# superlinear-ai/raglite

Measured on AMD Instinct MI355X. Metric: queries/sec, MaxSim 32x1M d=1024 exact top-100, higher is better.
Workload: dtype f32 in / f32 scores: candidate chunks found with the fp16 hi halves of corpus and queries (1 x v_mfma_f32_16x16x32_f16 per multiply, f32 accumulate, rigorous error bound), their scores by v_mfma_f32_16x16x4_f32 (exact f32 products); full-precision fallback: 3 x v_mfma_f32_16x16x32_f16 on hi+lo pairs

## Files before the change

raglite_amd/csrc/maxsim_pp.hip:

```cpp
#include <cstdio>
#include <cstdlib>
#include <utility>

#include "common.h"
#include "pp_schedule.h"
#include "scratch_layout.h"

namespace rl {

typedef float f32x4 __attribute__((ext_vector_type(4)));
typedef _Float16 h16x8 __attribute__((ext_vector_type(8)));

namespace {
constexpr int PP_RT = 128;
constexpr int PP_NBLK = PP_RT / 16;
constexpr int PP_QPP = 16;
constexpr int PP_DC = 8;
constexpr int PP_LC = 6;
constexpr int PP_CSLOT = PP_NBLK * 1024;
constexpr int PP_STAGE = 1536;
constexpr int PP_LDS = PP_DC * PP_CSLOT + 16 * PP_STAGE * 4;

__device__ __forceinline__ int64_t pp_uniform_i64(int64_t v) {
    const uint32_t lo = __builtin_amdgcn_readfirstlane((uint32_t)(uint64_t)v);
    const uint32_t hi = __builtin_amdgcn_readfirstlane((uint32_t)((uint64_t)v >> 32));
    return (int64_t)(((uint64_t)hi << 32) | lo);
}

enum { PP_HINT_NONE = 0, PP_HINT_NT = 1, PP_HINT_SC1 = 2 };
template <bool NT>
__device__ __forceinline__ void pp_dma(uint32_t lds, const char* src, uint32_t lane16, int hint) {
    const uint32_t l = __builtin_amdgcn_readfirstlane(lds);
    const char* const p = reinterpret_cast<const char*>(pp_uniform_i64(reinterpret_cast<int64_t>(src)));
#ifdef RAGLITE_EXPERIMENTS
    if (!NT && hint == PP_HINT_SC1) {
        asm volatile("s_mov_b32 m0, %0\n\ts_nop 0\n\tglobal_load_lds_dwordx4 %1, %2 sc1" ::"s"(l), "v"(lane16), "s"(p) : "memory", "m0");
        return;
    }
    if (NT || hint == PP_HINT_NT)
#else
    if constexpr (NT)
#endif
        asm volatile("s_mov_b32 m0, %0\n\ts_nop 0\n\tglobal_load_lds_dwordx4 %1, %2 nt" ::"s"(l), "v"(lane16), "s"(p) : "memory", "m0");
    else
        asm volatile("s_mov_b32 m0, %0\n\ts_nop 0\n\tglobal_load_lds_dwordx4 %1, %2" ::"s"(l), "v"(lane16), "s"(p) : "memory", "m0");
}

template <int OFF>
__device__ __forceinline__ void pp_read(f32x4& dst, uint32_t addr) {
    asm volatile("ds_read_b128 %0, %1 offset:%2" : "=v"(dst) : "v"(addr), "n"(OFF) : "memory");
}
__device__ __forceinline__ void pp_pin(f32x4& a, f32x4& b, f32x4& c, f32x4& d) { asm volatile("" : "+v"(a), "+v"(b), "+v"(c), "+v"(d)); }
typedef float f32x16s __attribute__((ext_vector_type(16)));
__device__ __forceinline__ f32x16s pp_sload16(const float* p) {
    f32x16s v;
    const float* const u = reinterpret_cast<const float*>(pp_uniform_i64(reinterpret_cast<int64_t>(p)));
    asm volatile("s_load_dwordx16 %0, %1, 0x0\n\ts_waitcnt lgkmcnt(0)" : "=s"(v) : "s"(u) : "memory");
    return v;
}
__device__ __forceinline__ h16x8 pp_h(const f32x4& v) {
    h16x8 r;
    __builtin_memcpy(&r, &v, 16);
    return r;
}
}

struct PpRows {
    const float* tau;
    const float* q_unscale;
    const float* q_sumsq;
    const float* row_norm;
    const float* blk_minmax;
    int32_t B, QT, metric;
    float* cand_scores; int32_t* cand_ids; uint32_t* cand_cnt; uint32_t* overflow; int32_t cap;
    uint2* log; int32_t log_cap;
    int32_t tile_begin, tile_count;
    float* S; int64_t ld_s; int32_t stride;
    int32_t xcd_passes, dma_hint;
};

template <int DBG, int MODE, bool ROWNORM>
__global__ __launch_bounds__(512, 2) void maxsim_pp_kernel(const char* __restrict__ planes, int64_t n_rows, int32_t nslab,
                                                           const char* __restrict__ qfrag, const float* __restrict__ qmeta, int32_t n_q,
                                                           const int32_t* __restrict__ row_to_chunk, const int64_t* __restrict__ chunk_offsets,
                                                           const uint32_t* __restrict__ ends_bits, float* __restrict__ out, int64_t out_stride,
                                                           float inv_e_scale, const uint32_t* __restrict__ run_if, PpRows rs) {
    constexpr bool ROWS = MODE == 2, SCORES = MODE == 1, GROUPS = ROWS || SCORES;
    __shared__ __attribute__((aligned(16))) char smem[PP_LDS];
    if (run_if && __builtin_amdgcn_readfirstlane((int)*run_if) == 0) return;
    const int lane = threadIdx.x & 63;
    const int wv = wave_id();
    int64_t G = gridDim.x, b = blockIdx.x;
    int qt = (int)blockIdx.y;
    if constexpr (!GROUPS) {
        const int32_t passes = (n_q + PP_QPP - 1) / PP_QPP;
        const PpSlot m = gridDim.y > 1 ? pp_schedule((int32_t)blockIdx.x, (int32_t)blockIdx.y, (int32_t)gridDim.x, (int32_t)gridDim.y, passes)
                                       : pp_schedule_affine((int32_t)blockIdx.x, (int32_t)gridDim.x, passes, rs.xcd_passes);
        G = __builtin_amdgcn_readfirstlane(m.ranges);
        b = __builtin_amdgcn_readfirstlane(m.range);
        qt = __builtin_amdgcn_readfirstlane(m.pass);
    }
    auto boundary = [&](int64_t t) -> int64_t {
        if (t <= 0) return 0;
        if (t >= n_rows) return n_rows;
        const int32_t c = row_to_chunk[t];
        const int64_t c0 = chunk_offsets[c], c1 = chunk_offsets[c + 1];
        return c0 == t ? t : c1;
    };
    int32_t r_lo = 0, r_hi = 0, nt_rows = 0;
    if constexpr (!GROUPS) {
        r_lo = (int32_t)pp_uniform_i64(boundary((n_rows * b) / G));
        r_hi = (int32_t)pp_uniform_i64((b + 1 == G) ? n_rows : boundary((n_rows * (b + 1)) / G));
        if (r_hi <= r_lo) return;
    } else {
        const int64_t Tr = rs.tile_count;
        const int64_t t0 = (Tr * b) / G, t1 = (Tr * (b + 1)) / G;
        nt_rows = (int32_t)(t1 - t0);
        if (nt_rows <= 0) return;
        r_lo = (int32_t)((rs.tile_begin + t0) * PP_RT);
        r_hi = (int32_t)n_rows;
    }
    const int32_t org = r_lo & ~15;
    const int nt = GROUPS ? nt_rows : (r_hi - org + PP_RT - 1) / PP_RT;
    auto tile_blk = [&](int t) __attribute__((always_inline)) -> int32_t {
        if constexpr (SCORES) {
            const int32_t o = (org >> 7) + t;
            return ((o >> 1) * 2 * rs.stride + (o & 1)) * PP_NBLK;
        } else {
            return (org >> 4) + t * PP_NBLK;
        }
    };
    const int q_base = GROUPS ? 0 : PP_QPP * qt;
    const int total = nt * nslab;
    const int32_t last_blk = (int32_t)((n_rows + 15) >> 4) - 1;
    const uint32_t lds_base = (uint32_t)reinterpret_cast<uintptr_t>((__attribute__((address_space(3))) char*)smem);
    const uint32_t lane16 = 16u * lane;

    const bool has0 = q_base + 2 * wv < n_q, has1 = q_base + 2 * wv + 1 < n_q;
    int ql0 = PP_QPP * qt + 2 * wv, ql1 = PP_QPP * qt + 2 * wv + 1;
    ql0 = ql0 < n_q ? ql0 : n_q - 1;
    ql1 = ql1 < n_q ? ql1 : n_q - 1;
    const char* const qp0 = qfrag + pp_uniform_i64((int64_t)ql0 * nslab * 4096);
    const char* const qp1 = qfrag + pp_uniform_i64((int64_t)ql1 * nslab * 4096);
    int qr_s = 0;
    auto issue_qregs = [&](f32x4 (&qn)[4]) __attribute__((always_inline)) {
        if constexpr (!(DBG & 32)) {
            const char* const a0 = reinterpret_cast<const char*>(pp_uniform_i64(reinterpret_cast<int64_t>(qp0 + (int64_t)qr_s * 4096)));
            const char* const a1 = reinterpret_cast<const char*>(pp_uniform_i64(reinterpret_cast<int64_t>(qp1 + (int64_t)qr_s * 4096)));
            asm volatile("global_load_dwordx4 %0, %2, %3\n\tglobal_load_dwordx4 %1, %2, %3 offset:2048"
                         : "=&v"(qn[0]), "=&v"(qn[1]) : "v"(lane16), "s"(a0) : "memory");
            asm volatile("global_load_dwordx4 %0, %2, %3\n\tglobal_load_dwordx4 %1, %2, %3 offset:2048"
                         : "=&v"(qn[2]), "=&v"(qn[3]) : "v"(lane16), "s"(a1) : "memory");
            if (++qr_s == nslab) qr_s = 0;
        }
    };
    int fc_s = 0, fc_r = 0, fc_slot = 0;
    const int dma_hint = GROUPS ? 0 : rs.dma_hint;
    const int32_t blk_org = (org >> 4) + wv;
    const int64_t slab_bytes = (int64_t)nslab * 1024;
    auto issue_c = [&]() __attribute__((always_inline)) {
        if constexpr (!(DBG & 16)) {
            const int t = fc_r < nt ? fc_r : nt - 1;
            int32_t blk = SCORES ? tile_blk(t) + wv : blk_org + t * PP_NBLK;
            blk = blk < last_blk ? blk : last_blk;
            const char* src = planes + pp_uniform_i64((int64_t)blk * slab_bytes + (int64_t)fc_s * 1024);
            pp_dma<GROUPS>(lds_base + (uint32_t)(fc_slot * PP_CSLOT + wv * 1024), src, lane16, dma_hint);
        }
        if (++fc_s == nslab) { fc_s = 0; ++fc_r; }
        fc_slot = fc_slot + 1 == PP_DC ? 0 : fc_slot + 1;
    };

    f32x4 acc[2][2][PP_NBLK];
#pragma unroll
    for (int q = 0; q < 2; ++q)
#pragma unroll
        for (int qb = 0; qb < 2; ++qb)
#pragma unroll
            for (int a = 0; a < PP_NBLK; ++a) acc[q][qb][a] = (f32x4){0.f, 0.f, 0.f, 0.f};

    f32x4 ef[PP_NBLK];
    f32x4 qA[4], qB[4];
    int c_slot = 0;
    const uint32_t rd_c = lds_base + lane16;
    auto read_slab = [&](auto A_) __attribute__((always_inline)) {
        constexpr int a = decltype(A_)::value;
        if constexpr (!(DBG & 8)) pp_read<a * 1024>(ef[a], rd_c + (uint32_t)(c_slot * PP_CSLOT));
    };
    auto mfma_group = [&](f32x4 (&q)[4], auto A_) __attribute__((always_inline)) {
        constexpr int A = decltype(A_)::value;
        if constexpr (!(DBG & 2)) {
            acc[0][0][A] = __builtin_amdgcn_mfma_f32_16x16x32_f16(pp_h(ef[A]), pp_h(q[0]), acc[0][0][A], 0, 0, 0);
            acc[0][1][A] = __builtin_amdgcn_mfma_f32_16x16x32_f16(pp_h(ef[A]), pp_h(q[1]), acc[0][1][A], 0, 0, 0);
            acc[1][0][A] = __builtin_amdgcn_mfma_f32_16x16x32_f16(pp_h(ef[A]), pp_h(q[2]), acc[1][0][A], 0, 0, 0);
            acc[1][1][A] = __builtin_amdgcn_mfma_f32_16x16x32_f16(pp_h(ef[A]), pp_h(q[3]), acc[1][1][A], 0, 0, 0);
        }
    };

    const int fG = lane >> 4, fb = (lane >> 2) & 3, ft = lane & 3;
    const int my_row = (ft >> 1) + 2 * (fb & 1) + 4 * (fb >> 1) + 8 * (fG & 1);
    const uint32_t my_bit = 1u << my_row, my_below = my_bit - 1u;
    float run = -INFINITY;
    uint32_t prev_last_end = 1;
    int32_t ord_run = GROUPS ? 0 : __builtin_amdgcn_readfirstlane(row_to_chunk[org]);
    const int e_q = fG >> 1;
    const bool e_has = !GROUPS && (e_q == 0 ? has0 : has1) && (ft & 1) == 0;
    const float e_unscale = e_has ? qmeta[2 * (q_base + 2 * wv + e_q)] * inv_e_scale : 0.f;
    [[maybe_unused]] float* const o_buf = reinterpret_cast<float*>(smem + PP_DC * PP_CSLOT) + (2 * wv + e_q) * PP_STAGE;
    [[maybe_unused]] const int32_t ord_lo = !GROUPS ? __builtin_amdgcn_readfirstlane(row_to_chunk[r_lo]) : 0;
    [[maybe_unused]] int32_t own_cnt = 0, own_flushed = 0;
    [[maybe_unused]] auto flush_out = [&]() __attribute__((always_inline)) {
        if constexpr (!GROUPS) {
            const int n = own_cnt - own_flushed;
            asm volatile("s_waitcnt lgkmcnt(0)" ::: "memory");
            const float* const b0 = reinterpret_cast<const float*>(smem + PP_DC * PP_CSLOT) + (2 * wv) * PP_STAGE;
            float* const g0 = out + (int64_t)(q_base + 2 * wv) * out_stride + ord_lo + own_flushed;
            if (has0)
                for (int i = lane; i < n; i += 64) g0[i] = b0[i];
            if (has1)
                for (int i = lane; i < n; i += 64) g0[out_stride + i] = b0[PP_STAGE + i];
            own_flushed = own_cnt;
            asm volatile("s_waitcnt vmcnt(0)" ::: "memory");
        }
    };
    const uint64_t odd_pairs = 0xccccccccccccccccull;
    auto swap32 = [](float& x, float& y) __attribute__((always_inline)) {
        const auto r = __builtin_amdgcn_permlane32_swap(__float_as_uint(x), __float_as_uint(y), false, false);
        x = __uint_as_float(r[0]);
        y = __uint_as_float(r[1]);
    };
    auto swap16 = [](float& x, float& y) __attribute__((always_inline)) {
        const auto r = __builtin_amdgcn_permlane16_swap(__float_as_uint(x), __float_as_uint(y), false, false);
        x = __uint_as_float(r[0]);
        y = __uint_as_float(r[1]);
    };
    auto zero_block = [&](auto A_) __attribute__((always_inline)) {
        constexpr int a = decltype(A_)::value;
#pragma unroll
        for (int q = 0; q < 2; ++q)
#pragma unroll
            for (int qb = 0; qb < 2; ++qb) acc[q][qb][a] = (f32x4){0.f, 0.f, 0.f, 0.f};
    };
    [[maybe_unused]] auto block_epilogue_maxsim = [&](auto A_, int T) __attribute__((always_inline)) {
        constexpr int a = decltype(A_)::value;
        const int32_t base = org + T * PP_RT + 16 * a;
        const uint32_t E = (ends_bits[base >> 5] >> (base & 16)) & 0xffffu;
        float z[16];
#pragma unroll
        for (int r = 0; r < 16; ++r) z[r] = acc[r >> 3][(r >> 2) & 1][a][r & 3];
#pragma unroll
        for (int u = 0; u < 4; ++u) { swap32(z[u], z[8 + u]); swap32(z[4 + u], z[12 + u]); }
#pragma unroll
        for (int u = 0; u < 4; ++u) { swap16(z[u], z[4 + u]); swap16(z[8 + u], z[12 + u]); }
        uint64_t saved;
        asm volatile(
            "s_mov_b64 %[sv], exec\n\t"
            "s_bitcmp1_b32 %[ple], 0\n\ts_cselect_b64 exec, 0, -1\n\tv_max_f32 %[z0], %[z0], %[run]\n\t"
            "s_bitcmp1_b32 %[E], 0\n\ts_cselect_b64 exec, 0, -1\n\tv_max_f32 %[z1], %[z1], %[z0]\n\t"
            "s_bitcmp1_b32 %[E], 1\n\ts_cselect_b64 exec, 0, -1\n\tv_max_f32 %[z2], %[z2], %[z1]\n\t"
            "s_bitcmp1_b32 %[E], 2\n\ts_cselect_b64 exec, 0, -1\n\tv_max_f32 %[z3], %[z3], %[z2]\n\t"
            "s_bitcmp1_b32 %[E], 3\n\ts_cselect_b64 exec, 0, -1\n\tv_max_f32 %[z4], %[z4], %[z3]\n\t"
            "s_bitcmp1_b32 %[E], 4\n\ts_cselect_b64 exec, 0, -1\n\tv_max_f32 %[z5], %[z5], %[z4]\n\t"
            "s_bitcmp1_b32 %[E], 5\n\ts_cselect_b64 exec, 0, -1\n\tv_max_f32 %[z6], %[z6], %[z5]\n\t"
            "s_bitcmp1_b32 %[E], 6\n\ts_cselect_b64 exec, 0, -1\n\tv_max_f32 %[z7], %[z7], %[z6]\n\t"
            "s_bitcmp1_b32 %[E], 7\n\ts_cselect_b64 exec, 0, -1\n\tv_max_f32 %[z8], %[z8], %[z7]\n\t"
            "s_bitcmp1_b32 %[E], 8\n\ts_cselect_b64 exec, 0, -1\n\tv_max_f32 %[z9], %[z9], %[z8]\n\t"
            "s_bitcmp1_b32 %[E], 9\n\ts_cselect_b64 exec, 0, -1\n\tv_max_f32 %[z10], %[z10], %[z9]\n\t"
            "s_bitcmp1_b32 %[E], 10\n\ts_cselect_b64 exec, 0, -1\n\tv_max_f32 %[z11], %[z11], %[z10]\n\t"
            "s_bitcmp1_b32 %[E], 11\n\ts_cselect_b64 exec, 0, -1\n\tv_max_f32 %[z12], %[z12], %[z11]\n\t"
            "s_bitcmp1_b32 %[E], 12\n\ts_cselect_b64 exec, 0, -1\n\tv_max_f32 %[z13], %[z13], %[z12]\n\t"
            "s_bitcmp1_b32 %[E], 13\n\ts_cselect_b64 exec, 0, -1\n\tv_max_f32 %[z14], %[z14], %[z13]\n\t"
            "s_bitcmp1_b32 %[E], 14\n\ts_cselect_b64 exec, 0, -1\n\tv_max_f32 %[z15], %[z15], %[z14]\n\t"
            "s_mov_b64 exec, %[sv]"
            : [sv] "=&s"(saved), [z0] "+v"(z[0]), [z1] "+v"(z[1]), [z2] "+v"(z[2]), [z3] "+v"(z[3]), [z4] "+v"(z[4]), [z5] "+v"(z[5]),
              [z6] "+v"(z[6]), [z7] "+v"(z[7]), [z8] "+v"(z[8]), [z9] "+v"(z[9]), [z10] "+v"(z[10]), [z11] "+v"(z[11]), [z12] "+v"(z[12]),
              [z13] "+v"(z[13]), [z14] "+v"(z[14]), [z15] "+v"(z[15])
            : [run] "v"(run), [E] "s"(E), [ple] "s"(prev_last_end)
            : "scc");
        run = z[15];
        prev_last_end = (E >> 15) & 1u;
        float s8[8];
#pragma unroll
        for (int k = 0; k < 8; ++k) {
            swap16(z[k], z[k + 8]);
            s8[k] = z[k] + z[k + 8];
        }
        float t0, t1, w;
        asm volatile(
            "s_nop 1\n\t"
            "v_add_f32_dpp %[s0], %[s0], %[s0] row_ror:8 row_mask:0xf bank_mask:0x3\n\t"
            "v_add_f32_dpp %[s1], %[s1], %[s1] row_ror:8 row_mask:0xf bank_mask:0x3\n\t"
            "v_add_f32_dpp %[s2], %[s2], %[s2] row_ror:8 row_mask:0xf bank_mask:0x3\n\t"
            "v_add_f32_dpp %[s3], %[s3], %[s3] row_ror:8 row_mask:0xf bank_mask:0x3\n\t"
            "v_add_f32_dpp %[s0], %[s4], %[s4] row_ror:8 row_mask:0xf bank_mask:0xc\n\t"
            "v_add_f32_dpp %[s1], %[s5], %[s5] row_ror:8 row_mask:0xf bank_mask:0xc\n\t"
            "v_add_f32_dpp %[s2], %[s6], %[s6] row_ror:8 row_mask:0xf bank_mask:0xc\n\t"
            "v_add_f32_dpp %[s3], %[s7], %[s7] row_ror:8 row_mask:0xf bank_mask:0xc\n\t"
            "v_add_f32_dpp %[s0], %[s0], %[s0] row_shl:4 row_mask:0xf bank_mask:0x5\n\t"
            "v_add_f32_dpp %[s1], %[s1], %[s1] row_shl:4 row_mask:0xf bank_mask:0x5\n\t"
            "v_add_f32_dpp %[s0], %[s2], %[s2] row_shr:4 row_mask:0xf bank_mask:0xa\n\t"
            "v_add_f32_dpp %[s1], %[s3], %[s3] row_shr:4 row_mask:0xf bank_mask:0xa\n\t"
            "s_nop 1\n\t"
            "v_add_f32_dpp %[t0], %[s0], %[s0] quad_perm:[2,3,0,1] row_mask:0xf bank_mask:0xf\n\t"
            "v_add_f32_dpp %[t1], %[s1], %[s1] quad_perm:[2,3,0,1] row_mask:0xf bank_mask:0xf\n\t"
            "v_cndmask_b32_e64 %[w], %[t0], %[t1], %[odd]\n\t"
            "s_nop 1\n\t"
            "v_add_f32_dpp %[w], %[w], %[w] quad_perm:[1,0,3,2] row_mask:0xf bank_mask:0xf"
            : [s0] "+v"(s8[0]), [s1] "+v"(s8[1]), [s2] "+v"(s8[2]), [s3] "+v"(s8[3]), [t0] "=&v"(t0), [t1] "=&v"(t1), [w] "=&v"(w)
            : [s4] "v"(s8[4]), [s5] "v"(s8[5]), [s6] "v"(s8[6]), [s7] "v"(s8[7]), [odd] "s"(odd_pairs));
        int32_t lo = r_lo - base, hi = r_hi - base;
        lo = lo < 0 ? 0 : lo;
        hi = hi < 0 ? 0 : hi;
        asm("" : "+s"(lo), "+s"(hi));
        lo = lo > 16 ? 16 : lo;
        hi = hi > 16 ? 16 : hi;
        uint32_t EM = E & ((1u << hi) - 1u) & ~((1u << lo) - 1u);
        asm("" : "+s"(EM));
        if (EM != 0u) {
            if ((EM & my_bit) && e_has) o_buf[ord_run - ord_lo - own_flushed + __builtin_popcount(E & my_below)] = w * e_unscale;
            own_cnt += __builtin_popcount(EM);
        }
        ord_run += __builtin_popcount(E);
        zero_block(A_);
    };

    [[maybe_unused]] float T4x = INFINITY;
    [[maybe_unused]] uint32_t ncand = 0;
    constexpr uint32_t LOG_CAP = PP_STAGE;
    [[maybe_unused]] uint2* const l_log = reinterpret_cast<uint2*>(smem + PP_DC * PP_CSLOT) + wv * LOG_CAP;
    [[maybe_unused]] uint32_t ncand_out = 0;
    [[maybe_unused]] uint2* const my_log = ROWS ? rs.log + (((size_t)blockIdx.y * gridDim.x + blockIdx.x) * 8 + wv) * (size_t)rs.log_cap : nullptr;
    [[maybe_unused]] const bool cosine = GROUPS && rs.metric == SCAN_COSINE;
    [[maybe_unused]] float Ux = 0.f, Rx = 0.f;
    if constexpr (SCORES) {
        const int c = lane >> 4;
        const int32_t q = (16 * qt + 2 * wv + (c >> 1)) * 32 + 16 * (c & 1) + (lane & 15);
        const int32_t qc = q < rs.B ? q : rs.B - 1;
        Ux = q < rs.B ? rs.q_unscale[qc] * inv_e_scale : 0.f;
        Rx = cosine ? 1.0f / sqrtf(rs.q_sumsq[qc]) : 1.0f;
    }
    if constexpr (ROWS) {
        const int c = lane >> 4;
        const int32_t q = (16 * qt + 2 * wv + (c >> 1)) * 32 + 16 * (c & 1) + (lane & 15);
        const int32_t qc = q < rs.B ? q : rs.B - 1;
        const float us = rs.q_unscale[qc] * inv_e_scale;
        const float tq = rs.tau[qc];
        const bool bad = q < rs.B && !(tq > -INFINITY);
        const float slack = 1e-5f * fmaxf(1.0f, fabsf(tq));
        const float t_dot = cosine ? (tq - slack) * sqrtf(rs.q_sumsq[qc]) : (tq - 1.0f) - slack;
        T4x = q < rs.B ? (t_dot - fabsf(t_dot) * 1e-6f) / us : INFINITY;
        if (__builtin_amdgcn_ballot_w64(bad) != 0 && lane == 0) *rs.overflow = 1u;
    }
    [[maybe_unused]] auto rows_thresholds = [&](float (&tq4)[4]) __attribute__((always_inline)) {
        uint32_t b;
        asm volatile("v_mbcnt_lo_u32_b32 %0, -1, 0\n\tv_mbcnt_hi_u32_b32 %0, -1, %0" : "=v"(b));
        b = (b & 15u) << 2;
#pragma unroll
        for (int c = 0; c < 4; ++c)
            tq4[c] = __int_as_float(__builtin_amdgcn_ds_bpermute((int)(((uint32_t)c << 6) | b), __float_as_int(T4x)));
    };
    [[maybe_unused]] auto block_epilogue_rows = [&](auto A_, int T, const float (&tq4)[4], float nmin, float nmax) __attribute__((always_inline)) {
        constexpr int a = decltype(A_)::value;
        const int32_t base = org + T * PP_RT + 16 * a;
        if (base < (int32_t)n_rows) {
            uint32_t lane_code = ((uint32_t)(lane & 15) << 7) | (uint32_t)(4 * (lane >> 4));
            asm volatile("" : "+v"(lane_code));
            float t4[4];
#pragma unroll
            for (int c = 0; c < 4; ++c) t4[c] = tq4[c];
            if (cosine) {
                nmin *= 0.999999f;
                nmax *= 1.000001f;
#pragma unroll
                for (int c = 0; c < 4; ++c) t4[c] = fminf(t4[c] * nmin, t4[c] * nmax);
            }
            const uint32_t code_a = ((uint32_t)T << 13) | (uint32_t)(16 * a);
            if constexpr (ROWNORM) {
                float top4[4];
                bool any_hit = false;
#pragma unroll
                for (int c = 0; c < 4; ++c) {
                    const f32x4 v4 = acc[c >> 1][c & 1][a];
                    top4[c] = fmaxf(fmaxf(v4[0], v4[1]), fmaxf(v4[2], v4[3]));
                    any_hit |= __builtin_amdgcn_ballot_w64(top4[c] >= t4[c]) != 0ull;
                }
                float nv0 = 1.f, nv1 = 1.f, nv2 = 1.f, nv3 = 1.f;
                const bool row_norms = cosine && base + 16 <= (int32_t)n_rows;
                if (any_hit && row_norms) {
                    const f32x16s nr = pp_sload16(rs.row_norm + base);
                    const int gq = lane >> 4;
                    nv0 = gq == 0 ? nr[0] : gq == 1 ? nr[4] : gq == 2 ? nr[8] : nr[12];
                    nv1 = gq == 0 ? nr[1] : gq == 1 ? nr[5] : gq == 2 ? nr[9] : nr[13];
                    nv2 = gq == 0 ? nr[2] : gq == 1 ? nr[6] : gq == 2 ? nr[10] : nr[14];
                    nv3 = gq == 0 ? nr[3] : gq == 1 ? nr[7] : gq == 2 ? nr[11] : nr[15];
                }
#pragma unroll
                for (int c = 0; c < 4; ++c) {
                    const f32x4 v4 = acc[c >> 1][c & 1][a];
                    if (__builtin_amdgcn_ballot_w64(top4[c] >= t4[c]) != 0ull) {
                        float r0 = v4[0], r1 = v4[1], r2 = v4[2], r3 = v4[3];
                        const float tc = tq4[c];
                        float n0 = nv0, n1 = nv1, n2 = nv2, n3 = nv3;
                        if (cosine && !row_norms) n0 = n1 = n2 = n3 = tc >= 0.f ? nmin : nmax;
                        uint32_t code = (code_a + ((uint32_t)c << 11)) | lane_code;
#pragma nounroll
                        for (int u = 0; u < 4; ++u) {
                            const float tn = tc * n0;
                            const bool pass = r0 >= fminf(tn * 0.999999f, tn * 1.000001f);
                            const uint64_t mask = __builtin_amdgcn_ballot_w64(pass);
                            if (mask != 0ull) {
                                const uint32_t pos = ncand + __builtin_amdgcn_mbcnt_hi((uint32_t)(mask >> 32), __builtin_amdgcn_mbcnt_lo((uint32_t)mask, 0u));
                                if (pass && pos - ncand_out < LOG_CAP) l_log[pos - ncand_out] = make_uint2(__float_as_uint(r0), code);
                                ncand += (uint32_t)__builtin_popcountll(mask);
                            }
                            r0 = r1; r1 = r2; r2 = r3;
                            n0 = n1; n1 = n2; n2 = n3;
                            ++code;
                            asm volatile("" : "+v"(r0), "+v"(code), "+v"(n0));
                        }
                    }
                }
            } else {
    #pragma unroll
                for (int c = 0; c < 4; ++c) {
                    const f32x4 v4 = acc[c >> 1][c & 1][a];
                    const float top = fmaxf(fmaxf(v4[0], v4[1]), fmaxf(v4[2], v4[3]));
                    if (__builtin_amdgcn_ballot_w64(top >= t4[c]) != 0ull) {
                        float r0 = v4[0], r1 = v4[1], r2 = v4[2], r3 = v4[3];
                        uint32_t code = (code_a + ((uint32_t)c << 11)) | lane_code;
    #pragma nounroll
                        for (int u = 0; u < 4; ++u) {
                            const bool pass = r0 >= t4[c];
                            const uint64_t mask = __builtin_amdgcn_ballot_w64(pass);
                            if (mask != 0ull) {
                                const uint32_t pos = ncand + __builtin_amdgcn_mbcnt_hi((uint32_t)(mask >> 32), __builtin_amdgcn_mbcnt_lo((uint32_t)mask, 0u));
                                if (pass && pos - ncand_out < LOG_CAP) l_log[pos - ncand_out] = make_uint2(__float_as_uint(r0), code);
                                ncand += (uint32_t)__builtin_popcountll(mask);
                            }
                            r0 = r1; r1 = r2; r2 = r3;
                            ++code;
                            asm volatile("" : "+v"(r0), "+v"(code));
                        }
                    }
                }
            }
        }
        zero_block(A_);
    };
    [[maybe_unused]] auto block_epilogue_scores = [&](auto A_, int T, const float (&us4)[4], const float (&rq4)[4], uint32_t n_op) __attribute__((always_inline)) {
        constexpr int a = decltype(A_)::value;
        const int32_t o = (org >> 7) + T;
        const int32_t base = (tile_blk(T) + a) * 16;
        const int64_t col = (int64_t)(o >> 1) * 256 + (o & 1) * 128 + 16 * a;
        const int gq = lane >> 4;
        float rn[4] = {1.f, 1.f, 1.f, 1.f};
        if (cosine && base < (int32_t)n_rows) {
            const f32x16s nr = pp_sload16(rs.row_norm + base);
            rn[0] = 1.0f / (gq == 0 ? nr[0] : gq == 1 ? nr[4] : gq == 2 ? nr[8] : nr[12]);
            rn[1] = 1.0f / (gq == 0 ? nr[1] : gq == 1 ? nr[5] : gq == 2 ? nr[9] : nr[13]);
            rn[2] = 1.0f / (gq == 0 ? nr[2] : gq == 1 ? nr[6] : gq == 2 ? nr[10] : nr[14]);
            rn[3] = 1.0f / (gq == 0 ? nr[3] : gq == 1 ? nr[7] : gq == 2 ? nr[11] : nr[15]);
        }
        const int32_t left = (int32_t)n_rows - (base + 4 * gq);
#pragma unroll
        for (int c = 0; c < 4; ++c) {
            const f32x4 v4 = acc[c >> 1][c & 1][a];
            f32x4 o4;
#pragma unroll
            for (int u = 0; u < 4; ++u) {
                const float d = v4[u] * us4[c];
                float v = cosine ? 1.0f - (1.0f - d * rn[u] * rq4[c]) : 1.0f + d;
                o4[u] = u < left ? v : -INFINITY;
            }
            const int32_t q = (16 * qt + 2 * wv + (c >> 1)) * 32 + 16 * (c & 1) + (int32_t)n_op;
            if (q < rs.B) *reinterpret_cast<f32x4*>(rs.S + (int64_t)q * rs.ld_s + col + 4 * gq) = o4;
        }
        zero_block(A_);
    };
    [[maybe_unused]] auto dump_log = [&]() __attribute__((always_inline)) {
        if constexpr (ROWS) {
            uint32_t n = ncand - ncand_out;
            if (n > LOG_CAP) {
                if (lane == 0) *rs.overflow = 1u;
                n = LOG_CAP;
            }
            asm volatile("s_waitcnt lgkmcnt(0)" ::: "memory");
            for (uint32_t i = lane; i < n; i += 64)
                if (ncand_out + i < (uint32_t)rs.log_cap) my_log[ncand_out + i] = l_log[i];
            ncand_out = ncand;
            asm volatile("s_waitcnt vmcnt(0)" ::: "memory");
        }
    };
    [[maybe_unused]] auto flush_rows = [&]() __attribute__((always_inline)) {
        if constexpr (ROWS) {
            if (ncand > (uint32_t)rs.log_cap) {
                if (lane == 0) *rs.overflow = 1u;
                ncand = (uint32_t)rs.log_cap;
            }
            const int mode = rs.metric;
            for (uint32_t i = lane; i < ncand; i += 64) {
                const uint2 rec = my_log[i];
                const uint32_t m = rec.y;
                const int T = (int)(m >> 13), c = (int)((m >> 11) & 3u), n = (int)((m >> 7) & 15u), r = (int)(m & 127u);
                const int32_t q = (16 * qt + 2 * wv + (c >> 1)) * 32 + 16 * (c & 1) + n, row = org + T * PP_RT + r;
                if (q >= rs.B || row >= (int32_t)n_rows) continue;
                const float d = __uint_as_float(rec.x) * (rs.q_unscale[q] * inv_e_scale);
                float v = d;
                if (mode == SCAN_COSINE) v = 1.0f - (1.0f - d / (rs.row_norm[row] * sqrtf(rs.q_sumsq[q])));
                else if (mode == SCAN_DOT) v = 1.0f + d;
                if (!(v >= rs.tau[q])) continue;
                const uint32_t slot = atomicAdd(rs.cand_cnt + q, 1u);
                if (slot < (uint32_t)rs.cap) {
                    rs.cand_scores[(int64_t)q * rs.cap + slot] = v;
                    rs.cand_ids[(int64_t)q * rs.cap + slot] = row;
                } else {
                    *rs.overflow = 1u;
                }
            }
        }
    };

    int c_s = 0, c_r = 0;
#define PP_I(N) std::integral_constant<int, N>{}
    auto tile_end = [&]() __attribute__((always_inline)) {
        if constexpr (DBG & 128) return;
        if (c_s == nslab - 1) {
            if constexpr (SCORES) {
                float us4[4], rq4[4];
                uint32_t bl;
                asm volatile("v_mbcnt_lo_u32_b32 %0, -1, 0\n\tv_mbcnt_hi_u32_b32 %0, -1, %0" : "=v"(bl));
                bl = (bl & 15u) << 2;
#pragma unroll
                for (int c = 0; c < 4; ++c) {
                    us4[c] = __int_as_float(__builtin_amdgcn_ds_bpermute((int)(((uint32_t)c << 6) | bl), __float_as_int(Ux)));
                    rq4[c] = __int_as_float(__builtin_amdgcn_ds_bpermute((int)(((uint32_t)c << 6) | bl), __float_as_int(Rx)));
                }
                [&]<int... A>(std::integer_sequence<int, A...>) {
                    (block_epilogue_scores(std::integral_constant<int, A>{}, c_r, us4, rq4, bl >> 2), ...);
                }(std::make_integer_sequence<int, PP_NBLK>{});
            } else if constexpr (ROWS) {
                float tq4[4];
                rows_thresholds(tq4);
                f32x16s mm = {};
                if (cosine) mm = pp_sload16(rs.blk_minmax + 2 * ((org + c_r * PP_RT) >> 4));
                [&]<int... A>(std::integer_sequence<int, A...>) {
                    (block_epilogue_rows(std::integral_constant<int, A>{}, c_r, tq4, mm[2 * A], mm[2 * A + 1]), ...);
                }(std::make_integer_sequence<int, PP_NBLK>{});
                if (ncand - ncand_out > LOG_CAP / 2) dump_log();
            } else {
                [&]<int... A>(std::integer_sequence<int, A...>) { (block_epilogue_maxsim(std::integral_constant<int, A>{}, c_r), ...); }
                (std::make_integer_sequence<int, PP_NBLK>{});
                if (own_cnt - own_flushed > PP_STAGE - PP_RT) flush_out();
            }
        }
    };
    auto slab = [&](f32x4 (&q)[4], f32x4 (&qn)[4], auto LAG_) __attribute__((always_inline)) {
        constexpr bool LAG = decltype(LAG_)::value;
        auto G = [&](auto A_) __attribute__((always_inline)) { mfma_group(q, A_); };
        auto R = [&](auto A_) __attribute__((always_inline)) { read_slab(A_); };
        issue_qregs(qn);
        issue_c();
        __builtin_amdgcn_sched_barrier(0);
        if constexpr (!LAG) {
            G(PP_I(0)); R(PP_I(0)); __builtin_amdgcn_sched_barrier(0);
            G(PP_I(1)); R(PP_I(1)); __builtin_amdgcn_sched_barrier(0);
            G(PP_I(2)); R(PP_I(2)); __builtin_amdgcn_sched_barrier(0);
            G(PP_I(3)); R(PP_I(3)); __builtin_amdgcn_sched_barrier(0);
            asm volatile("s_waitcnt lgkmcnt(4)" ::: "memory");
        } else {
            G(PP_I(0)); __builtin_amdgcn_sched_barrier(0);
            G(PP_I(1)); R(PP_I(0)); __builtin_amdgcn_sched_barrier(0);
            G(PP_I(2)); R(PP_I(1)); __builtin_amdgcn_sched_barrier(0);
            G(PP_I(3)); R(PP_I(2)); __builtin_amdgcn_sched_barrier(0);
            asm volatile("s_waitcnt lgkmcnt(3)" ::: "memory");
        }
        pp_pin(ef[4], ef[5], ef[6], ef[7]);
        asm volatile("s_barrier" ::: "memory");
        __builtin_amdgcn_sched_barrier(0);
        if constexpr (!LAG) {
            G(PP_I(4)); R(PP_I(4)); __builtin_amdgcn_sched_barrier(0);
            G(PP_I(5)); R(PP_I(5)); __builtin_amdgcn_sched_barrier(0);
            G(PP_I(6)); R(PP_I(6)); __builtin_amdgcn_sched_barrier(0);
            G(PP_I(7)); R(PP_I(7)); __builtin_amdgcn_sched_barrier(0);
        } else {
            G(PP_I(4)); R(PP_I(3)); __builtin_amdgcn_sched_barrier(0);
            G(PP_I(5)); R(PP_I(4)); __builtin_amdgcn_sched_barrier(0);
            G(PP_I(6)); R(PP_I(5)); __builtin_amdgcn_sched_barrier(0);
            G(PP_I(7)); R(PP_I(6)); __builtin_amdgcn_sched_barrier(0);
            R(PP_I(7)); __builtin_amdgcn_sched_barrier(0);
        }
        c_slot = c_slot + 1 == PP_DC ? 0 : c_slot + 1;
        tile_end();
        if (++c_s == nslab) { c_s = 0; ++c_r; }
    };
    auto landed = [&](f32x4 (&qn)[4]) __attribute__((always_inline)) {
        asm volatile("s_waitcnt lgkmcnt(4)" ::: "memory");
        asm volatile("s_waitcnt vmcnt(1)" ::: "memory");
        pp_pin(ef[0], ef[1], ef[2], ef[3]);
        pp_pin(qn[0], qn[1], qn[2], qn[3]);
    };

    for (int i = 0; i < PP_LC; ++i) issue_c();
    issue_qregs(qA);
    asm volatile("s_waitcnt vmcnt(0)\n\ts_barrier" ::: "memory");
    [&]<int... A>(std::integer_sequence<int, A...>) { (read_slab(std::integral_constant<int, A>{}), ...); }
    (std::make_integer_sequence<int, PP_NBLK>{});
    c_slot = 1;
    landed(qA);
    auto main_loop = [&](auto LAG_) __attribute__((always_inline)) {
        for (int g = 0; g < total; g += 2) {
            slab(qA, qB, LAG_);
            landed(qB);
            if (g + 1 < total) {
                slab(qB, qA, LAG_);
                landed(qA);
            }
        }
    };
#undef PP_I
    if (wv < 4) main_loop(std::false_type{});
    else main_loop(std::true_type{});
    asm volatile("s_waitcnt vmcnt(0)" ::: "memory");
    dump_log();
    flush_rows();
    flush_out();
    if constexpr (DBG & 128) {
        if (n_q > 1000000) {
            f32x4 t = (f32x4){0.f, 0.f, 0.f, 0.f};
#pragma unroll
            for (int q = 0; q < 2; ++q)
#pragma unroll
                for (int qb = 0; qb < 2; ++qb)
#pragma unroll
                    for (int a = 0; a < PP_NBLK; ++a) t += acc[q][qb][a];
            out[lane] = (t[0] + t[1]) + (t[2] + t[3]);
        }
    }
}

int launch_maxsim_pp(const void* image, int64_t n_rows, int32_t dim, const void* qbuf, int32_t n_queries, int32_t first, int32_t n_q,
                     int32_t nq, const int32_t* row_to_chunk, const int64_t* chunk_offsets, const uint32_t* ends_bits, float* out,
                     int64_t out_stride, int n_cu, hipStream_t s, float split_scale, const uint32_t* run_if, int schedule, int xcd_passes) {
    if (nq < 1 || nq > 32 || n_q < 1 || n_q > PP_QPP * 4096 || n_rows < 1 || first < 0 || first + n_q > n_queries) return RL_ERR_UNSUPPORTED;
    if (dim % 32 || dim < 256 || !(split_scale > 0.f) || !image || !ends_bits) return RL_ERR_UNSUPPORTED;
    const int32_t nslab = dim / 32;
    const char* qfrag = static_cast<const char*>(qbuf) + (size_t)first * nslab * 4096;
    QueryPlanes L;
    L.lay(Carver(const_cast<void*>(qbuf)), n_queries, dim);
    const float* qmeta = L.meta + 2 * (size_t)first;
    const int64_t tiles = (n_rows + PP_RT - 1) / PP_RT;
    const int64_t gx = std::max<int64_t>(1, std::min<int64_t>(n_cu > 0 ? n_cu : 256, tiles)), passes = (n_q + PP_QPP - 1) / PP_QPP;
    const dim3 grid = schedule == 1 ? dim3((unsigned)(gx * passes)) : dim3((unsigned)gx, (unsigned)passes), blk(512);
    PpRows rs{};
    rs.xcd_passes = schedule == 1 ? xcd_passes : 8;
#define RL_PP_LAUNCH(DBG_)                                                                                                                 \
    hipLaunchKernelGGL((maxsim_pp_kernel<DBG_, 0, false>), grid, blk, 0, s, static_cast<const char*>(image), n_rows, nslab, qfrag, qmeta, n_q, row_to_chunk, \
                       chunk_offsets, ends_bits, out, out_stride, 1.0f / split_scale, run_if, rs)
#ifdef RAGLITE_EXPERIMENTS
    const int force_hint = std::getenv("RAGLITE_PP_HINT") ? std::atoi(std::getenv("RAGLITE_PP_HINT")) : -1;
    if (force_hint >= PP_HINT_NONE && force_hint <= PP_HINT_SC1) rs.dma_hint = force_hint;
    static const int dbg = std::getenv("RAGLITE_PP_DBG") ? std::atoi(std::getenv("RAGLITE_PP_DBG")) : 0;
    if (dbg == 2) RL_PP_LAUNCH(2);
    else if (dbg == 128) RL_PP_LAUNCH(128);
    else if (dbg == 136) RL_PP_LAUNCH(136);
    else if (dbg == 144) RL_PP_LAUNCH(144);
    else if (dbg == 160) RL_PP_LAUNCH(160);
    else if (dbg == 184) RL_PP_LAUNCH(184);
    else RL_PP_LAUNCH(0);
#else
    RL_PP_LAUNCH(0);
#endif
#undef RL_PP_LAUNCH
    RL_HIP(hipGetLastError());
    return RL_OK;
}

__global__ __launch_bounds__(256) void block_norm_minmax_kernel(const float* __restrict__ row_norm, int64_t n_rows, int64_t n_blocks,
                                                                 float* __restrict__ out) {
    const int64_t blk = (int64_t)blockIdx.x * 256 + threadIdx.x;
    if (blk >= n_blocks) return;
    float mn = INFINITY, mx = 0.f;
    for (int i = 0; i < 16; ++i) {
        const int64_t r = blk * 16 + i;
        if (r < n_rows) { const float v = row_norm[r]; mn = fminf(mn, v); mx = fmaxf(mx, v); }
    }
    out[2 * blk] = mn;
    out[2 * blk + 1] = mx;
}

int launch_pp_rows_sample(const void* image, int64_t n_rows, int32_t dim, int32_t nb, float* scratch, const float* row_norm, int mode, float* S,
                          int64_t ld_s, int32_t stride, int n_cu, hipStream_t s, float split_scale) {
    if (nb < 1 || n_rows < 1 || dim % 32 || dim < 256 || !(split_scale > 0.f) || !image || !S || stride < 1) return RL_ERR_UNSUPPORTED;
    if (mode != SCAN_COSINE && mode != SCAN_DOT) return RL_ERR_UNSUPPORTED;
    if (mode == SCAN_COSINE && !row_norm) return RL_ERR_INVALID;
    if ((ld_s & 255) || (reinterpret_cast<uintptr_t>(S) & 15)) return RL_ERR_UNSUPPORTED;
    const int32_t nslab = dim / 32, groups = (nb + 31) / 32;
    ScoreQueries L;
    L.lay(Carver(scratch), nb, dim);
    float *const frag = L.frag, *const unscale = L.unscale, *const qss = L.q_sumsq;
    const int64_t grid_cu = n_cu > 0 ? n_cu : 256;
    const int64_t T256 = (n_rows + 255) / 256, Tv = (T256 + stride - 1) / stride;
    if (Tv * 256 != ld_s) return RL_ERR_INVALID;
    PpRows rs{};
    rs.tile_begin = 0;
    rs.tile_count = (int32_t)(2 * Tv);
    rs.q_unscale = unscale; rs.q_sumsq = qss; rs.row_norm = row_norm; rs.B = nb; rs.QT = (groups + PP_QPP - 1) / PP_QPP; rs.metric = mode;
    rs.S = S; rs.ld_s = ld_s; rs.stride = stride;
    if (rs.QT > grid_cu) return RL_ERR_UNSUPPORTED;
    const int64_t gx = std::max<int64_t>(1, std::min<int64_t>(grid_cu / rs.QT, 2 * Tv));
    hipLaunchKernelGGL((maxsim_pp_kernel<0, 1, false>), dim3((unsigned)gx, (unsigned)rs.QT), dim3(512), 0, s, static_cast<const char*>(image), n_rows,
                       nslab, reinterpret_cast<const char*>(frag), nullptr, groups, nullptr, nullptr, nullptr, nullptr, (int64_t)0,
                       1.0f / split_scale, nullptr, rs);
    RL_HIP(hipGetLastError());
    return RL_OK;
}

size_t pp_rows_scratch_bytes(int64_t n_rows, int32_t nb, int n_cu, int32_t expected_per_query, int32_t* log_cap_out) {
    const int64_t grid = n_cu > 0 ? n_cu : 256;
    int64_t cap = ((int64_t)expected_per_query * nb * 4) / (grid * 8) + 1;
    cap = std::max<int64_t>(4096, (cap + 1023) & ~int64_t(1023));
    cap = std::min<int64_t>(cap, int64_t(1) << 19);
    if (log_cap_out) *log_cap_out = (int32_t)cap;
    const size_t blocks = (size_t)((n_rows + 15) / 16);
    return (size_t)grid * 8 * (size_t)cap * sizeof(uint2) + blocks * 2 * sizeof(float) + 256;
}

int launch_pp_rows_pass(const void* image, int64_t n_rows, int32_t dim, int32_t nb, float* scratch, const float* row_norm, int mode,
                        const CandArgs* cand, void* work, int32_t log_cap, int n_cu, hipStream_t s, float split_scale, int64_t tile_begin,
                        int64_t tile_count, bool norms_ready, bool row_norm_test) {
    if (nb < 1 || n_rows < 1 || dim % 32 || dim < 256 || !(split_scale > 0.f) || !image || !cand || !work) return RL_ERR_UNSUPPORTED;
    if (mode != SCAN_COSINE && mode != SCAN_DOT) return RL_ERR_UNSUPPORTED;
    if (mode == SCAN_COSINE && !row_norm) return RL_ERR_INVALID;
    if (cand->tau_stride != 1) return RL_ERR_UNSUPPORTED;
    const int32_t nslab = dim / 32, groups = (nb + 31) / 32;
    ScoreQueries L;
    L.lay(Carver(scratch), nb, dim);
    float *const frag = L.frag, *const unscale = L.unscale, *const qss = L.q_sumsq;
    const int64_t grid_cu = n_cu > 0 ? n_cu : 256;
    const int64_t Tr_all = (n_rows + PP_RT - 1) / PP_RT;
    if (tile_count < 0) tile_count = Tr_all - tile_begin;
    if (tile_begin < 0 || tile_count < 1 || tile_begin + tile_count > Tr_all) return RL_ERR_INVALID;
    const int64_t Tr = tile_count;
    PpRows rs{};
    rs.tile_begin = (int32_t)tile_begin;
    rs.tile_count = (int32_t)tile_count;
    rs.tau = cand->tau; rs.q_unscale = unscale; rs.q_sumsq = qss; rs.row_norm = row_norm; rs.B = nb; rs.QT = (groups + PP_QPP - 1) / PP_QPP;
    rs.metric = mode; rs.cand_scores = cand->scores; rs.cand_ids = cand->ids; rs.cand_cnt = cand->cnt; rs.overflow = cand->overflow; rs.cap = cand->cap;
    rs.log = static_cast<uint2*>(work);
    rs.log_cap = log_cap;
    if (rs.QT > grid_cu || Tr_all + 2 >= (int64_t(1) << 19)) return RL_ERR_UNSUPPORTED;
    float* blk_mm = reinterpret_cast<float*>(static_cast<char*>(work) + (size_t)grid_cu * 8 * (size_t)log_cap * sizeof(uint2));
    rs.blk_minmax = blk_mm;
    if (mode == SCAN_COSINE && !norms_ready) {
        const int64_t n_blocks = (n_rows + 15) / 16;
        hipLaunchKernelGGL(block_norm_minmax_kernel, dim3((unsigned)((n_blocks + 255) / 256)), dim3(256), 0, s, row_norm, n_rows, n_blocks, blk_mm);
    }
    const int64_t gx = std::max<int64_t>(1, std::min<int64_t>(grid_cu / rs.QT, Tr));
    const dim3 grid((unsigned)gx, (unsigned)rs.QT), blk(512);
#define RL_PP_ROWS(DBG_, RN_)                                                                                                             \
    hipLaunchKernelGGL((maxsim_pp_kernel<DBG_, 2, RN_>), grid, blk, 0, s, static_cast<const char*>(image), n_rows, nslab, reinterpret_cast<const char*>(frag), \
                       nullptr, groups, nullptr, nullptr, nullptr, nullptr, (int64_t)0, 1.0f / split_scale, nullptr, rs)
#ifdef RAGLITE_EXPERIMENTS
    static const int dbg = std::getenv("RAGLITE_PP_ROWS_DBG") ? std::atoi(std::getenv("RAGLITE_PP_ROWS_DBG")) : 0;
    if (dbg == 128) RL_PP_ROWS(128, false);
    else if (row_norm_test) RL_PP_ROWS(0, true);
    else RL_PP_ROWS(0, false);
#else
    if (row_norm_test) RL_PP_ROWS(0, true);
    else RL_PP_ROWS(0, false);
#endif
#undef RL_PP_ROWS
    RL_HIP(hipGetLastError());
    return RL_OK;
}

__global__ __launch_bounds__(512, 2) void mfma_f16_rate_kernel(float* __restrict__ out, int32_t iters) {
    const uint32_t lane = threadIdx.x & 63u, wv = threadIdx.x >> 6;
    f32x4 ef[8], qf[4];
    auto frag = [&](uint32_t tag) {
        f32x4 v;
#pragma unroll
        for (int i = 0; i < 4; ++i) {
            uint32_t h = (lane * 0x9E3779B1u) ^ ((tag * 4u + (uint32_t)i + 1u) * 0x85EBCA77u) ^ (wv * 0xC2B2AE3Du) ^ (blockIdx.x * 0x27D4EB2Fu);
            h ^= h >> 15; h *= 0x2C1B3C6Du; h ^= h >> 12;
            const uint32_t lo = (h & 0x83FFu) | (((h >> 10) & 3u) + 11u) << 10, hi = ((h >> 16) & 0x83FFu) | (((h >> 26) & 3u) + 11u) << 10;
            v[i] = __uint_as_float(lo | (hi << 16));
        }
        return v;
    };
#pragma unroll
    for (int a = 0; a < 8; ++a) ef[a] = frag(a);
#pragma unroll
    for (int c = 0; c < 4; ++c) qf[c] = frag(8 + c);
    f32x4 acc[8][4];
#pragma unroll
    for (int a = 0; a < 8; ++a)
#pragma unroll
        for (int c = 0; c < 4; ++c) acc[a][c] = (f32x4){0.f, 0.f, 0.f, 0.f};
    for (int32_t t = 0; t < iters; ++t) {
#pragma unroll
        for (int a = 0; a < 8; ++a)
#pragma unroll
            for (int c = 0; c < 4; ++c) acc[a][c] = __builtin_amdgcn_mfma_f32_16x16x32_f16(pp_h(ef[a]), pp_h(qf[c]), acc[a][c], 0, 0, 0);
    }
    f32x4 t4 = (f32x4){0.f, 0.f, 0.f, 0.f};
#pragma unroll
    for (int a = 0; a < 8; ++a)
#pragma unroll
        for (int c = 0; c < 4; ++c) t4 += acc[a][c];
    out[(size_t)blockIdx.x * 512 + threadIdx.x] = (t4[0] + t4[1]) + (t4[2] + t4[3]);
}

int launch_mfma_f16_rate(float* out, int n_cu, int32_t iters, hipStream_t s, double* flops) {
    if (!out || iters < 1) return RL_ERR_INVALID;
    const int grid = n_cu > 0 ? n_cu : 256;
    hipLaunchKernelGGL(mfma_f16_rate_kernel, dim3((unsigned)grid), dim3(512), 0, s, out, iters);
    RL_HIP(hipGetLastError());
    if (flops) *flops = (double)grid * 8.0 * (double)iters * 32.0 * (2.0 * 16 * 16 * 32);
    return RL_OK;
}

}
```

Baseline: 18030.

## Add tile-structured main loop mode with scalar-loaded end bits and fused accumulator reset

Adds a MODE 3 (TILES) variant of the MaxSim kernel whose main loop iterates explicitly over row tiles and slab pairs instead of a flat slab counter with per-slab tile_end checks. The chunk-end bitmask for each tile is fetched once with a scalar s_load_dwordx8 rather than per-block vector loads, and the first slab of each tile uses an inline-asm MFMA with zero accumulator input in place of a separate zero_block pass. The intent is to remove per-slab bookkeeping and the epilogue load and zeroing overhead. This mode becomes the default whenever nslab is even, with the old path kept as a fallback.

After: 18860, median of 6. 4.6% higher.

```diff
diff --git a/raglite_amd/csrc/maxsim_pp.hip b/raglite_amd/csrc/maxsim_pp.hip
--- a/raglite_amd/csrc/maxsim_pp.hip
+++ b/raglite_amd/csrc/maxsim_pp.hip
@@ -86,6 +86,8 @@
                                                            const uint32_t* __restrict__ ends_bits, float* __restrict__ out, int64_t out_stride,
                                                            float inv_e_scale, const uint32_t* __restrict__ run_if, PpRows rs) {
     constexpr bool ROWS = MODE == 2, SCORES = MODE == 1, GROUPS = ROWS || SCORES;
+    constexpr bool TILES = MODE == 3;
+    static_assert(!TILES || DBG == 0, "the timing skeletons keep the slab-counting loop");
     __shared__ __attribute__((aligned(16))) char smem[PP_LDS];
     if (run_if && __builtin_amdgcn_readfirstlane((int)*run_if) == 0) return;
     const int lane = threadIdx.x & 63;
@@ -186,9 +188,14 @@
         constexpr int a = decltype(A_)::value;
         if constexpr (!(DBG & 8)) pp_read<a * 1024>(ef[a], rd_c + (uint32_t)(c_slot * PP_CSLOT));
     };
-    auto mfma_group = [&](f32x4 (&q)[4], auto A_) __attribute__((always_inline)) {
+    auto mfma_group = [&](f32x4 (&q)[4], auto A_, auto FIRST_) __attribute__((always_inline)) {
         constexpr int A = decltype(A_)::value;
-        if constexpr (!(DBG & 2)) {
+        constexpr bool FIRST = decltype(FIRST_)::value;
+        if constexpr (FIRST && !(DBG & 2)) {
+#pragma unroll
+            for (int c = 0; c < 4; ++c)
+                asm volatile("v_mfma_f32_16x16x32_f16 %0, %1, %2, 0" : "+v"(acc[c >> 1][c & 1][A]) : "v"(ef[A]), "v"(q[c]));
+        } else if constexpr (!(DBG & 2)) {
             acc[0][0][A] = __builtin_amdgcn_mfma_f32_16x16x32_f16(pp_h(ef[A]), pp_h(q[0]), acc[0][0][A], 0, 0, 0);
             acc[0][1][A] = __builtin_amdgcn_mfma_f32_16x16x32_f16(pp_h(ef[A]), pp_h(q[1]), acc[0][1][A], 0, 0, 0);
             acc[1][0][A] = __builtin_amdgcn_mfma_f32_16x16x32_f16(pp_h(ef[A]), pp_h(q[2]), acc[1][0][A], 0, 0, 0);
@@ -214,10 +221,12 @@
             asm volatile("s_waitcnt lgkmcnt(0)" ::: "memory");
             const float* const b0 = reinterpret_cast<const float*>(smem + PP_DC * PP_CSLOT) + (2 * wv) * PP_STAGE;
             float* const g0 = out + (int64_t)(q_base + 2 * wv) * out_stride + ord_lo + own_flushed;
+            int ln = lane;
+            if constexpr (TILES) asm volatile("" : "+v"(ln));
             if (has0)
-                for (int i = lane; i < n; i += 64) g0[i] = b0[i];
+                for (int i = ln; i < n; i += 64) g0[i] = b0[i];
             if (has1)
-                for (int i = lane; i < n; i += 64) g0[out_stride + i] = b0[PP_STAGE + i];
+                for (int i = ln; i < n; i += 64) g0[out_stride + i] = b0[PP_STAGE + i];
             own_flushed = own_cnt;
             asm volatile("s_waitcnt vmcnt(0)" ::: "memory");
         }
@@ -240,10 +249,24 @@
 #pragma unroll
             for (int qb = 0; qb < 2; ++qb) acc[q][qb][a] = (f32x4){0.f, 0.f, 0.f, 0.f};
     };
+    typedef uint32_t u32x8s __attribute__((ext_vector_type(8)));
+    [[maybe_unused]] u32x8s tile_ends = {};
+    [[maybe_unused]] const uint32_t ends_shift = (uint32_t)org & 16u;
+    [[maybe_unused]] auto pp_tile_ends = [&](int T) __attribute__((always_inline)) {
+        const uint32_t* const p = reinterpret_cast<const uint32_t*>(pp_uniform_i64(reinterpret_cast<int64_t>(ends_bits + ((org + T * PP_RT) >> 5))));
+        asm volatile("s_load_dwordx8 %0, %1, 0x0" : "=&s"(tile_ends) : "s"(p) : "memory");
+    };
+    [[maybe_unused]] auto tile_ends_of = [&](auto A_) __attribute__((always_inline)) -> uint32_t {
+        constexpr int a = decltype(A_)::value;
+        const uint64_t pair = ((uint64_t)tile_ends[a / 2 + 1] << 32) | tile_ends[a / 2];
+        return (uint32_t)(pair >> (ends_shift + 16u * (a & 1))) & 0xffffu;
+    };
     [[maybe_unused]] auto block_epilogue_maxsim = [&](auto A_, int T) __attribute__((always_inline)) {
         constexpr int a = decltype(A_)::value;
         const int32_t base = org + T * PP_RT + 16 * a;
-        const uint32_t E = (ends_bits[base >> 5] >> (base & 16)) & 0xffffu;
+        uint32_t E;
+        if constexpr (TILES) E = tile_ends_of(A_);
+        else E = (ends_bits[base >> 5] >> (base & 16)) & 0xffffu;
         float z[16];
 #pragma unroll
         for (int r = 0; r < 16; ++r) z[r] = acc[r >> 3][(r >> 2) & 1][a][r & 3];
@@ -320,7 +343,12 @@
             own_cnt += __builtin_popcount(EM);
         }
         ord_run += __builtin_popcount(E);
-        zero_block(A_);
+        if constexpr (!TILES) {
+            zero_block(A_);
+        } else {
+#pragma unroll
+            for (int r = 0; r < 16; ++r) acc[r >> 3][(r >> 2) & 1][a][r & 3] = z[r];
+        }
     };
 
     [[maybe_unused]] float T4x = INFINITY;
@@ -553,9 +581,9 @@
             }
         }
     };
-    auto slab = [&](f32x4 (&q)[4], f32x4 (&qn)[4], auto LAG_) __attribute__((always_inline)) {
+    auto slab = [&](f32x4 (&q)[4], f32x4 (&qn)[4], auto LAG_, auto FIRST_) __attribute__((always_inline)) {
         constexpr bool LAG = decltype(LAG_)::value;
-        auto G = [&](auto A_) __attribute__((always_inline)) { mfma_group(q, A_); };
+        auto G = [&](auto A_) __attribute__((always_inline)) { mfma_group(q, A_, FIRST_); };
         auto R = [&](auto A_) __attribute__((always_inline)) { read_slab(A_); };
         issue_qregs(qn);
         issue_c();
@@ -589,8 +617,10 @@
             R(PP_I(7)); __builtin_amdgcn_sched_barrier(0);
         }
         c_slot = c_slot + 1 == PP_DC ? 0 : c_slot + 1;
-        tile_end();
-        if (++c_s == nslab) { c_s = 0; ++c_r; }
+        if constexpr (!TILES) {
+            tile_end();
+            if (++c_s == nslab) { c_s = 0; ++c_r; }
+        }
     };
     auto landed = [&](f32x4 (&qn)[4]) __attribute__((always_inline)) {
         asm volatile("s_waitcnt lgkmcnt(4)" ::: "memory");
@@ -600,19 +630,45 @@
     };
 
     for (int i = 0; i < PP_LC; ++i) issue_c();
-    issue_qregs(qA);
-    asm volatile("s_waitcnt vmcnt(0)\n\ts_barrier" ::: "memory");
-    [&]<int... A>(std::integer_sequence<int, A...>) { (read_slab(std::integral_constant<int, A>{}), ...); }
-    (std::make_integer_sequence<int, PP_NBLK>{});
-    c_slot = 1;
-    landed(qA);
+    auto prologue_fragments = [&]() __attribute__((always_inline)) {
+        issue_qregs(qA);
+        asm volatile("s_waitcnt vmcnt(0)\n\ts_barrier" ::: "memory");
+        [&]<int... A>(std::integer_sequence<int, A...>) { (read_slab(std::integral_constant<int, A>{}), ...); }
+        (std::make_integer_sequence<int, PP_NBLK>{});
+        c_slot = 1;
+        landed(qA);
+    };
+    if constexpr (!TILES) prologue_fragments();
     auto main_loop = [&](auto LAG_) __attribute__((always_inline)) {
-        for (int g = 0; g < total; g += 2) {
-            slab(qA, qB, LAG_);
-            landed(qB);
-            if (g + 1 < total) {
-                slab(qB, qA, LAG_);
+        if constexpr (TILES) {
+            const int pairs = nslab >> 1;
+            prologue_fragments();
+            for (int t = 0; t < nt; ++t) {
+                pp_tile_ends(t);
+                slab(qA, qB, LAG_, std::true_type{});
+                landed(qB);
+                slab(qB, qA, LAG_, std::false_type{});
                 landed(qA);
+#pragma nounroll
+                for (int p = 1; p < pairs; ++p) {
+                    slab(qA, qB, LAG_, std::false_type{});
+                    landed(qB);
+                    slab(qB, qA, LAG_, std::false_type{});
+                    landed(qA);
+                }
+                asm volatile("s_waitcnt lgkmcnt(0)" : "+s"(tile_ends) : : "memory");
+                [&]<int... A>(std::integer_sequence<int, A...>) { (block_epilogue_maxsim(std::integral_constant<int, A>{}, t), ...); }
+                (std::make_integer_sequence<int, PP_NBLK>{});
+                if (own_cnt - own_flushed > PP_STAGE - PP_RT) flush_out();
+            }
+        } else {
+            for (int g = 0; g < total; g += 2) {
+                slab(qA, qB, LAG_, std::false_type{});
+                landed(qB);
+                if (g + 1 < total) {
+                    slab(qB, qA, LAG_, std::false_type{});
+                    landed(qA);
+                }
             }
         }
     };
@@ -652,24 +708,28 @@
     const dim3 grid = schedule == 1 ? dim3((unsigned)(gx * passes)) : dim3((unsigned)gx, (unsigned)passes), blk(512);
     PpRows rs{};
     rs.xcd_passes = schedule == 1 ? xcd_passes : 8;
-#define RL_PP_LAUNCH(DBG_)                                                                                                                 \
-    hipLaunchKernelGGL((maxsim_pp_kernel<DBG_, 0, false>), grid, blk, 0, s, static_cast<const char*>(image), n_rows, nslab, qfrag, qmeta, n_q, row_to_chunk, \
+#define RL_PP_LAUNCH(DBG_) RL_PP_LAUNCH_MODE(DBG_, 0)
+#define RL_PP_LAUNCH_MODE(DBG_, MODE_)                                                                                                     \
+    hipLaunchKernelGGL((maxsim_pp_kernel<DBG_, MODE_, false>), grid, blk, 0, s, static_cast<const char*>(image), n_rows, nslab, qfrag, qmeta, n_q, row_to_chunk, \
                        chunk_offsets, ends_bits, out, out_stride, 1.0f / split_scale, run_if, rs)
 #ifdef RAGLITE_EXPERIMENTS
     const int force_hint = std::getenv("RAGLITE_PP_HINT") ? std::atoi(std::getenv("RAGLITE_PP_HINT")) : -1;
     if (force_hint >= PP_HINT_NONE && force_hint <= PP_HINT_SC1) rs.dma_hint = force_hint;
-    static const int dbg = std::getenv("RAGLITE_PP_DBG") ? std::atoi(std::getenv("RAGLITE_PP_DBG")) : 0;
+    const int dbg = std::getenv("RAGLITE_PP_DBG") ? std::atoi(std::getenv("RAGLITE_PP_DBG")) : 0;
     if (dbg == 2) RL_PP_LAUNCH(2);
     else if (dbg == 128) RL_PP_LAUNCH(128);
     else if (dbg == 136) RL_PP_LAUNCH(136);
     else if (dbg == 144) RL_PP_LAUNCH(144);
     else if (dbg == 160) RL_PP_LAUNCH(160);
     else if (dbg == 184) RL_PP_LAUNCH(184);
-    else RL_PP_LAUNCH(0);
+    else if (dbg == 1 || nslab % 2) RL_PP_LAUNCH(0);
+    else RL_PP_LAUNCH_MODE(0, 3);
 #else
-    RL_PP_LAUNCH(0);
+    if (nslab % 2) RL_PP_LAUNCH(0);
+    else RL_PP_LAUNCH_MODE(0, 3);
 #endif
 #undef RL_PP_LAUNCH
+#undef RL_PP_LAUNCH_MODE
     RL_HIP(hipGetLastError());
     return RL_OK;
 }
```
